# google/deepconsensus

Hardware: NVIDIA H100
Metric: zmw_windows_per_sec (higher is better)
Workload: dtype bf16

## Files before the change

### deepconsensus_b200/csrc/engine.cu

```cuda
#include <cuda_bf16.h>
#include <cuda_runtime.h>
#include <math.h>
#include <stdarg.h>
#include <stdio.h>
#include <string.h>

#include <algorithm>
#include <cmath>
#include <functional>
#include <map>
#include <memory>
#include <string>
#include <vector>

#include "../../include/dcb200.h"
#include "../../include/dcb200_debug.h"
#include "kernels.h"

using namespace dcb;

namespace {

thread_local std::string g_create_error;

// ... 68 lines not shown

enum ProfKind { kProfEmbed, kProfRowGemm, kProfQkv, kProfAttention, kProfFfn, kProfHead, kProfKinds, kProfNone };

struct ProfRegion { cudaEvent_t start, end; ProfKind kind; };

}

struct dcb_engine {
  dcb_config cfg{};
  std::string err;
  int R = 0, L = 0, Lw = 0, E = 0, Epad = 0, echunks = 0;
  PackedLayout pl{};
  int chunk_tiles = 0, chunk_windows = 0;
  int num_sms = 132;
  cudaStream_t stream = nullptr;
  cudaStream_t copy_stream = nullptr;
  cudaStream_t out_stream = nullptr;
  struct Slot {
    DevBuf<float> d_rows;
    DevBuf<uint8_t> d_packed;
    DevBuf<uint8_t> d_bases, d_quals;
    DevBuf<float> d_probs, d_logits;
    DevBuf<int> d_status;
    int* h_status = nullptr;
    cudaEvent_t rows_ready = nullptr, ev0 = nullptr, ev1 = nullptr, done = nullptr;
    bool busy = false, used = false;
    int64_t ticket = -1;
    int launches = 0;
    std::vector<ProfRegion> prof;
    size_t prof_used = 0;
  } slots[2];
  int64_t next_ticket = 0;
  bool weights_loaded = false;
  bool debug = false;
  bool profile = false;
  float prof_ms[kProfKinds] = {};
  int prof_n[kProfKinds] = {};
  long long prof_ffn_tokens = 0;
  float last_ms = 0.f;
  int last_launches = 0;
  int last_chunk_tokens = 0;
  std::vector<EmbedTable> tables;
  std::vector<StrictEmbedRow> embed;
  int table_elems = 0;
  Weights w;
  DevBuf<__nv_bfloat16> d_embqkv;
  DevBuf<float> d_x;
  DevBuf<__nv_bfloat16> d_xb;
  DevBuf<__nv_bfloat16> d_att;
  DevBuf<__nv_bfloat16> d_hid;
  DevBuf<int> d_flow;
  uint32_t flow_stamp = 0;
  bool tile_flow = false;
  DevBuf<double> d_p10;
  DevBuf<float> d_dbg;
  DevBuf<__nv_bfloat16> d_dbg_op;
  struct Strict {
    DevBuf<float> emb, x, y, q, k, v, att, hid;
    int chunk_windows = 0;
  } strict;
  struct {
    DevBuf<uint8_t> bases, quals, seq, qual, names, fastq;
    DevBuf<int32_t> start, len, pos, name_off, outcome;
    DevBuf<int64_t> rec_off, win_off;
    DevBuf<double> avg_q;
  } st;
  struct { DevBuf<int16_t> bq; DevBuf<uint8_t> mask; DevBuf<double> avg; } sk;
  struct {
    DevBuf<uint8_t> ids, bases, quals; DevBuf<int16_t> bq; DevBuf<int32_t> dst; DevBuf<int64_t> src_off, dst_off; DevBuf<int> status;
  } fs;
  struct { DevBuf<float> probs, loss; DevBuf<uint8_t> labels, ccs, exact; DevBuf<int32_t> pred, ccs_counts; DevBuf<int> bad; } ev;
  struct { DevBuf<float> teacher, student, loss, grad; } ds;
  struct { DevBuf<float> probs, loss, grad, matches, dp; DevBuf<uint8_t> labels; } lg;
  struct { DevBuf<float> bias, logits, probs; DevBuf<uint8_t> bases, quals; } he;
  struct {
    DevBuf<PrepZmw> zmw;
    DevBuf<int32_t> meta, noni, gap, zmw_windows, window_pos, window_width, num_passes, list, wl;
    DevBuf<int64_t> ccs_off;
    DevBuf<float> sn;
    DevBuf<uint32_t> cigar;
    DevBuf<uint8_t> bases, pw, ip, ccs_bases, ccs_bq, spaced, overflow, ccs_ids, packed;
    DevBuf<int4> op_scan, zmw_out;
    DevBuf<int4> win_list, window;
    DevBuf<int16_t> out_bq, ccs_bq_full;
    DevBuf<uint8_t> ccs_ids_full;
    DevBuf<int32_t> label_meta;
    DevBuf<uint32_t> label_cigar;
    DevBuf<uint8_t> label_bases, labels, label_status;
    DevBuf<int4> label_scan;
    DevBuf<int32_t> eval_dst;
    DevBuf<uint8_t> keep;
    DevBuf<int> eval_count;
    std::vector<int32_t> width;
    DevBuf<int> status;
    PrepBatch batch{};
    int n_windows = -1;
  } fp;
  cudaEvent_t ev_eval0 = nullptr, ev_eval1 = nullptr;

  ~dcb_engine() {
    for (cudaStream_t s : {copy_stream, stream, out_stream})
      if (s) cudaStreamSynchronize(s);
    std::vector<cudaEvent_t> events = {ev_eval0, ev_eval1};
    for (Slot& sl : slots) {
      events.insert(events.end(), {sl.rows_ready, sl.ev0, sl.ev1, sl.done});
      for (const ProfRegion& r : sl.prof) events.insert(events.end(), {r.start, r.end});
// ... 480 lines not shown
  const uint32_t nstamps = 3 + 3 * (uint32_t)c.num_hidden_layers;
  if (flow && e->flow_stamp > UINT32_MAX - nstamps) {
    cudaMemsetAsync(e->d_flow, 0, e->chunk_tiles * sizeof(int), st);
    e->flow_stamp = 0;
  }
  auto next_flow = [&](bool advance = true) {
    TileFlow f{};
    if (flow) {
      f.flags = e->d_flow;
      f.status = d_status;
      f.wait = (int)e->flow_stamp;
      f.done = (int)(e->flow_stamp + 1);
      if (advance) ++e->flow_stamp;
    }
    return f;
  };
  int stage = 0;
  auto snap = [&]() {
    if (e->debug) {
      const size_t ximg = x_image_elems(), cw = (size_t)e->chunk_tiles * kTileM;
      cudaMemcpyAsync(e->d_dbg + (size_t)stage * e->chunk_tiles * ximg, e->d_x, T * ximg * sizeof(float), cudaMemcpyDeviceToDevice, st);
      size_t cols = 0;
      for (const DbgImage& im : dbg_images(e)) {
        if (im.stage == stage)
          cudaMemcpyAsync(e->d_dbg_op + cols * cw, im.src->p, (size_t)T * kTileM * im.width * sizeof(__nv_bfloat16),
                          cudaMemcpyDeviceToDevice, st);
        cols += im.width;
      }
    }
    ++stage;
  };
  rec.run(kProfEmbed, 1, [&] {
    launch_embed(rows_chunk, packed_chunk, e->pl, e->R, L, Lw, M, T, e->echunks, W.cols, W.rowmeta, W.tables,
                 e->table_elems, e->d_embqkv, d_status, next_flow(), st);
  });
  rec.run(kProfRowGemm, 1, [&] {
    launch_gemm_row(e->d_embqkv, W.wc, e->Epad / 16, 2 * (e->Epad / 16), T, row_epi(e, false, nullptr, 0, 0, true),
                    next_flow(), st);
  });
  snap();
  for (int n_ = 0; n_ < c.num_hidden_layers; ++n_) {
    const LayerDev& ld = W.layers[n_];
    if (Lw == kTileM) {
      rec.run(kProfAttention, 2, [&] {
        __nv_bfloat16* qkv = e->debug ? e->d_embqkv.p : nullptr;
        for (int half = 0; half < 2; ++half)
          launch_qkv_attention(half, e->d_xb, ld.wqkv, L, c.attn_win_size, T, qkv, e->d_att, next_flow(half == 1), st);
      });
    } else {
      rec.run(kProfQkv, 1, [&] { launch_gemm_qkv(e->d_xb, ld.wqkv, T, e->d_embqkv, st); });
      rec.run(kProfAttention, 1, [&] { launch_attention(e->d_embqkv, e->d_att, L, Lw, c.attn_win_size, bw, st); });
    }
    rec.run(kProfRowGemm, 1, [&] {
      launch_gemm_row(e->d_att, ld.wo, kDP / 16, 2 * (kDP / 16), T, row_epi(e, true, nullptr, n_, 1, false), next_flow(),
                      st);
    });
    snap();
    rec.run(kProfFfn, 2, [&] {
      const RowEpi epi = row_epi(e, true, ld.b2, n_ + 1, 0, false);
      __nv_bfloat16* hid = e->debug ? e->d_hid.p : nullptr;
      for (int half = 0; half < 2; ++half)
        launch_ffn(half, e->d_xb, ld.w1, ld.b1, ld.w2, c.filter_size, T, hid, epi, next_flow(half == 1), st);
    });
    if (e->profile) e->prof_ffn_tokens += (long long)bw * L;
    snap();
  }
  hp.x = e->d_x; hp.M = M; hp.L = L; hp.Lw = Lw;
  rec.run(kProfHead, 1, [&] { launch_head(hp, T, next_flow(), st); });
  e->last_chunk_tokens = M;
}

}

extern "C" {

const char* dcb_version(void) { return "dcb200 0.1.0 (sm_90a)"; }

const char* dcb_last_error(const dcb_engine* e) { return e ? e->err.c_str() : g_create_error.c_str(); }

int dcb_create(const dcb_config* cfg, dcb_engine** out) {
  if (!cfg || !out) return fail(nullptr, DCB_ERR_INVALID, "null argument");
  if (cfg->struct_size != (int32_t)sizeof(dcb_config))
    return fail(nullptr, DCB_ERR_INVALID, "dcb_config size mismatch: got %d, built with %zu",
                cfg->struct_size, sizeof(dcb_config));
  if (cfg->hidden_size != kD || cfg->num_heads != kHeads)
    return fail(nullptr, DCB_ERR_INVALID, "unsupported model: hidden_size=%d num_heads=%d (engine is built for %d/%d)",
                cfg->hidden_size, cfg->num_heads, kD, kHeads);
  if (!cfg->condense_transformer_input)
    return fail(nullptr, DCB_ERR_INVALID, "condense_transformer_input must be true");
  if (cfg->filter_size <= 0 || cfg->filter_size % kFFChunk || cfg->filter_size > 2048)
    return fail(nullptr, DCB_ERR_INVALID, "filter_size must be a multiple of %d and <= 2048", kFFChunk);
  if (cfg->max_passes <= 0 || cfg->max_length <= 0 || cfg->max_length > 256 || cfg->num_hidden_layers <= 0 ||
      cfg->max_batch <= 0)
    return fail(nullptr, DCB_ERR_INVALID, "bad max_passes/max_length(<=256)/num_hidden_layers/max_batch");
  if (cfg->precision != DCB_PRECISION_BF16 && cfg->precision != DCB_PRECISION_FP32 && cfg->precision != DCB_PRECISION_TF32X3)
    return fail(nullptr, DCB_ERR_INVALID, "precision must be DCB_PRECISION_BF16, DCB_PRECISION_FP32 or DCB_PRECISION_TF32X3");
  int ndev = 0;
  if (cudaGetDeviceCount(&ndev) != cudaSuccess || ndev == 0)
    return fail(nullptr, DCB_ERR_CUDA, "no CUDA device available (the dcb200 engine has no CPU fallback)");
  if (cfg->device < 0 || cfg->device >= ndev) return fail(nullptr, DCB_ERR_INVALID, "bad device ordinal %d", cfg->device);
  cudaDeviceProp prop;
  if (cudaGetDeviceProperties(&prop, cfg->device) != cudaSuccess || prop.major != 9)
    return fail(nullptr, DCB_ERR_CUDA, "device %d is not an sm_90 GPU (compute capability %d.%d)", cfg->device,
                prop.major, prop.minor);

  std::unique_ptr<dcb_engine> eng(new dcb_engine());
  dcb_engine* e = eng.get();
  e->cfg = *cfg;
  e->num_sms = prop.multiProcessorCount;
  e->L = cfg->max_length;
  e->Lw = e->L;
  bool align = true, tile_flow = true;
#ifdef DCB_DEV_SWITCHES
  if (const char* env = getenv("DCB_ALIGN")) align = atoi(env) != 0;
  if (const char* env = getenv("DCB_TILE_FLOW")) tile_flow = atoi(env) != 0;
#endif
  if (align && e->L <= kTileM) e->Lw = kTileM;
  e->tile_flow = tile_flow && e->Lw == kTileM;
  e->R = 4 * cfg->max_passes + (cfg->use_ccs_bq ? 6 : 5);
  e->pl = make_packed_layout(cfg->max_passes, cfg->max_length, cfg->use_ccs_bq ? 1 : 0);
  {
    auto table = [&](const char* layer, int vocab, int width) {
      const int off = (e->table_elems + 7) / 8 * 8;
      e->tables.push_back(EmbedTable{layer, vocab, width, off});
      e->table_elems = off + vocab * width;
      return e->tables.back();
    };
    auto rows = [&](const EmbedTable& tb, int n, float clip, int shift) {
      for (int r = 0; r < n; ++r) {
        e->embed.push_back(StrictEmbedRow{clip, shift, tb.vocab, tb.width, e->E, tb.off});
        e->E += tb.width;
      }
    };
    const int P = cfg->max_passes;
    const EmbedTable bases = table("bases_embedding_layer", kVocab, cfg->per_base_hidden_size);
    rows(bases, P, 0.f, 0);
    rows(table("pw_embedding_layer", cfg->pw_max + 1, cfg->pw_hidden_size), P, (float)cfg->pw_max, 0);
    rows(table("ip_embedding_layer", cfg->ip_max + 1, cfg->ip_hidden_size), P, (float)cfg->ip_max, 0);
    rows(table("strand_embedding_layer", cfg->strand_max + 1, cfg->strand_hidden_size), P, 0.f, 0);
    rows(bases, 1, 0.f, 0);
    if (cfg->use_ccs_bq)
      rows(table("ccs_base_quality_scores_embedding_layer", cfg->ccs_bq_max, cfg->ccs_bq_hidden_size), 1, 0.f, 1);
    rows(table("sn_embedding_layer", cfg->sn_max + 1, cfg->sn_hidden_size), 4, (float)cfg->sn_max, 0);
  }
  e->Epad = (e->E + 15) / 16 * 16;
  e->echunks = e->Epad / 8;
  const int ct = cfg->chunk_tiles > 0 ? cfg->chunk_tiles : 8 * e->num_sms;
  const int max_tiles = (int)(((int64_t)cfg->max_batch * e->Lw + kTileM - 1) / kTileM);
  e->chunk_windows = std::max(1, std::min(cfg->max_batch, ct * kTileM / e->Lw));
  e->chunk_tiles = std::min(max_tiles, (e->chunk_windows * e->Lw + kTileM - 1) / kTileM);

  const int rc = [&]() -> int {
    CU(e, cudaSetDevice(cfg->device));
    CU(e, cudaStreamCreateWithFlags(&e->stream, cudaStreamNonBlocking));
    CU(e, cudaStreamCreateWithFlags(&e->copy_stream, cudaStreamNonBlocking));
    CU(e, cudaStreamCreateWithFlags(&e->out_stream, cudaStreamNonBlocking));
    for (auto& sl : e->slots) {
      CU(e, cudaEventCreateWithFlags(&sl.rows_ready, cudaEventDisableTiming));
      CU(e, cudaEventCreate(&sl.ev0));
      CU(e, cudaEventCreate(&sl.ev1));
      CU(e, cudaEventCreateWithFlags(&sl.done, cudaEventDisableTiming));
      CU(e, cudaMallocHost(reinterpret_cast<void**>(&sl.h_status), sizeof(int)));
    }
    CU(e, cudaEventCreate(&e->ev_eval0));
    CU(e, cudaEventCreate(&e->ev_eval1));
    CU(e, kernels_init());
    CU(e, tf32x3_init());
    std::vector<double> p10(256);
// ... 1131 lines not shown
```

### deepconsensus_b200/csrc/kernels.cu

```cuda
#include "kernels.h"

#include <cuda_bf16.h>
#include <math.h>
#include <stdio.h>
#include <stdlib.h>

#include "head_finish.cuh"
#include "sm90.cuh"

namespace dcb {

__device__ __forceinline__ void pdl_launch_dependents() { asm volatile("griddepcontrol.launch_dependents;" ::: "memory"); }
__device__ __forceinline__ void pdl_wait() { asm volatile("griddepcontrol.wait;" ::: "memory"); }

__device__ __forceinline__ int ld_acquire_gpu(const int* p) {
  int v;
  asm volatile("ld.acquire.gpu.global.b32 %0, [%1];" : "=r"(v) : "l"(p) : "memory");
  return v;
}

__device__ __forceinline__ void tile_wait(const TileFlow& f, int tile) {
  if (!f.flags) return;
  if (ld_acquire_gpu(f.flags + tile) == f.wait) return;
  uint64_t t0, t;
// ... 80 lines not shown
    uint4* dst = reinterpret_cast<uint4*>(emb + ((size_t)tile * echunks + kc) * kTileM * 8) + r;
    *dst = val;
  }
  __syncthreads();
  if (threadIdx.x == 0) tile_done(flow, tile);
}

enum { EPI_QKV = 0, EPI_ROW = 1 };

template <int BN, int NCH, bool kAres>
struct GemmCfg {
  static constexpr int kNI = NCH * BN;
  static constexpr int kSK = 2;
  static constexpr int kABytesPerK = 2 * kTileM * 16;
  static constexpr int kBBytesPerK = 2 * kNI * 16;
  static constexpr int kStageBytes = kSK * ((kAres ? 0 : kABytesPerK) + kBBytesPerK);
  static constexpr int kStages = 8;
  static constexpr int kShortStages = 4;
  static constexpr int kLongK = 32;
  __host__ __device__ static constexpr int stages(int kstages) {
    return kAres || kstages >= kLongK ? kStages : kShortStages;
  }
  static constexpr int kMH = kAres ? 2 : 1;
  static constexpr int kATileBytes = (kDP / 16) * kABytesPerK;
  static constexpr int kAresBytes = kAres ? 2 * kATileBytes : 0;
  static constexpr int kThreads = 384;
  static constexpr int kVecBytes = kAres ? 0 : 3 * kDP * 4;
  __host__ __device__ static constexpr int smem_bytes(int nst) { return kAresBytes + nst * kStageBytes + 256 + kVecBytes; }
  static constexpr int kSmemBytes = smem_bytes(kStages);
  static_assert(kSmemBytes <= 232448, "over the sm_90 opt-in shared memory per block");
  static_assert((2 * kStages + 4) * 8 <= 256, "the mbarriers (full, empty, a_full, a_empty, turn[2]) fill 256 bytes");
};

template <int BN>
__device__ __forceinline__ void wgmma_bn(float (&d)[BN / 2], uint64_t a, uint64_t b, int acc);
template <>
__device__ __forceinline__ void wgmma_bn<144>(float (&d)[72], uint64_t a, uint64_t b, int acc) { wgmma_m64n144k16(d, a, b, acc); }
template <>
__device__ __forceinline__ void wgmma_bn<128>(float (&d)[64], uint64_t a, uint64_t b, int acc) { wgmma_m64n128k16(d, a, b, acc); }

__device__ __forceinline__ float quad_sum(float v) {
  v += __shfl_xor_sync(0xffffffffu, v, 1);
  v += __shfl_xor_sync(0xffffffffu, v, 2);
  return v;
}

__device__ __forceinline__ void row_vectors_to_smem(float* s_vec, const RowEpi& epi) {
  for (int i = threadIdx.x; i < kDP; i += blockDim.x) {
    if (epi.bias) s_vec[i] = epi.bias[i];
    if (epi.ln_g) { s_vec[kDP + i] = epi.ln_g[i]; s_vec[2 * kDP + i] = epi.ln_b[i]; }
  }
}

template <int BN, int NCH, bool kPe = true>
__device__ __forceinline__ void row_epilogue(float (&acc)[NCH][BN / 2], int tile, int row0, int q, const float* s_vec,
                                             const RowEpi& epi) {
  float* xt = epi.x + (size_t)tile * x_image_elems();
  const int xoff = ((q >> 1) * kTileM + row0) * 4 + 2 * (q & 1);
  const bool ln = epi.ln_g != nullptr;
#pragma unroll
  for (int h = 0; h < 2; ++h) {
    const int row = row0 + 8 * h;
    const int l = (tile * kTileM + row) % epi.L;
    float* xr = xt + xoff + 32 * h;
    const float* per = epi.pe_img ? epi.pe_img + xoff + 32 * h : epi.pe + (size_t)l * kDP + 2 * q;
    const int pe_stride = epi.pe_img ? kTileM : 1;
    float s1 = 0.f;
#pragma unroll
    for (int j = 0; j < NCH; ++j) {
      float2 ld[BN / 8];
      if (epi.has_xold) {
#pragma unroll
        for (int jj = 0; jj < BN / 8; ++jj)
          ld[jj] = *reinterpret_cast<const float2*>(xr + (j * BN + jj * 8) * kTileM);
#pragma unroll
        for (int jj = 0; jj < BN / 8; ++jj) {
          acc[j][jj * 4 + 2 * h] += ld[jj].x;
          acc[j][jj * 4 + 2 * h + 1] += ld[jj].y;
        }
      }
      if (kPe && epi.pe) {
#pragma unroll
        for (int jj = 0; jj < BN / 8; ++jj)
          ld[jj] = __ldg(reinterpret_cast<const float2*>(per + (size_t)(j * BN + jj * 8) * pe_stride));
      }
#pragma unroll
      for (int jj = 0; jj < BN / 8; ++jj) {
        const int col = j * BN + jj * 8 + 2 * q;
        float2 v = make_float2(acc[j][jj * 4 + 2 * h], acc[j][jj * 4 + 2 * h + 1]);
        if (epi.bias) {
          const float2 b = *reinterpret_cast<const float2*>(s_vec + col);
          v.x += b.x; v.y += b.y;
        }
        if (kPe && epi.pe) { v.x += ld[jj].x; v.y += ld[jj].y; }
        v.x = col < kD ? v.x : 0.f;
        v.y = col + 1 < kD ? v.y : 0.f;
        *reinterpret_cast<float2*>(xr + (j * BN + jj * 8) * kTileM) = v;
        acc[j][jj * 4 + 2 * h] = v.x;
        acc[j][jj * 4 + 2 * h + 1] = v.y;
        s1 += v.x + v.y;
      }
    }
    if (!epi.xb) continue;
    float mean = 0.f, rstd = 1.f;
    if (ln) {
      mean = quad_sum(s1) * (1.f / kD);
      float s2 = 0.f;
#pragma unroll
      for (int j = 0; j < NCH; ++j)
#pragma unroll
        for (int jj = 0; jj < BN / 8; ++jj) {
          const int col = j * BN + jj * 8 + 2 * q;
          const float d0 = col < kD ? acc[j][jj * 4 + 2 * h] - mean : 0.f;
          const float d1 = col + 1 < kD ? acc[j][jj * 4 + 2 * h + 1] - mean : 0.f;
          s2 += d0 * d0 + d1 * d1;
        }
      rstd = rsqrtf(quad_sum(s2) * (1.f / kD) + 1e-6f);
    }
    __nv_bfloat16* xb = epi.xb + (size_t)tile * act_image_elems(kDP) + row * 8 + 2 * q;
#pragma unroll
    for (int j = 0; j < NCH; ++j)
#pragma unroll
      for (int jj = 0; jj < BN / 8; ++jj) {
        const int col = j * BN + jj * 8 + 2 * q;
        float v0 = acc[j][jj * 4 + 2 * h], v1 = acc[j][jj * 4 + 2 * h + 1];
        if (ln) {
          v0 = col < kD ? (v0 - mean) * rstd * s_vec[kDP + col] + s_vec[2 * kDP + col] : 0.f;
          v1 = col + 1 < kD ? (v1 - mean) * rstd * s_vec[kDP + col + 1] + s_vec[2 * kDP + col + 1] : 0.f;
        }
        *reinterpret_cast<uint32_t*>(xb + (j * BN + jj * 8) * kTileM) = pack_bf16x2(v0, v1);
      }
  }
#pragma unroll
  for (int j = 0; j < NCH; ++j)
#pragma unroll
    for (int i = 0; i < BN / 2; ++i) acc[j][i] = 0.f;
}

template <int BN, int NCH, int EPI, bool kAres>
__global__ void __launch_bounds__(384, 1)
gemm_kernel(const __nv_bfloat16* __restrict__ a_img, const __nv_bfloat16* __restrict__ b_img, int a_ksteps, int ksteps,
            int ntiles,
            int ngroups, __nv_bfloat16* __restrict__ out_img, int out_chunks, RowEpi epi, TileFlow flow) {
  using Cfg = GemmCfg<BN, NCH, kAres>;
  static_assert(EPI != EPI_ROW || (Cfg::kNI == kDP && !kAres), "row epilogue needs the full 288-wide row");
  extern __shared__ __align__(1024) uint8_t smem[];
  uint8_t* a_res = smem;
  const int kstages = ksteps / Cfg::kSK;
  const int nst = Cfg::stages(kstages);
  uint8_t* stage_base = smem + Cfg::kAresBytes;
  uint64_t* full = reinterpret_cast<uint64_t*>(stage_base + nst * Cfg::kStageBytes);
  uint64_t* empty = full + nst;
  uint64_t* a_full = empty + nst;
  uint64_t* a_empty = a_full + 1;
  uint64_t* turn = a_empty + 1;
  float* s_vec = reinterpret_cast<float*>(stage_base + nst * Cfg::kStageBytes + 256);

  const int warp = threadIdx.x >> 5;
  const int lane = threadIdx.x & 31;
  if constexpr (EPI == EPI_ROW) row_vectors_to_smem(s_vec, epi);
  if (threadIdx.x == 0) {
    for (int i = 0; i < nst; ++i) {
      mbar_init(&full[i], 1);
      mbar_init(&empty[i], 256);
    }
    mbar_init(a_full, 1);
    mbar_init(a_empty, 256);
    mbar_init(&turn[0], 128);
    mbar_init(&turn[1], 128);
    mbar_fence_init();
  }
  __syncthreads();
  pdl_launch_dependents();

  const int nitems = kAres ? (ntiles + 1) / 2 : ntiles * ngroups;
  const int gper = kAres ? ngroups : 1;
  const size_t a_tile_bytes = (size_t)a_ksteps * Cfg::kABytesPerK;
  const size_t b_group_bytes = (size_t)ksteps * Cfg::kBBytesPerK;

  if (warp >= 8) {
    setmaxnreg_dec<40>();
    if (warp == 8 && lane == 0) {
      uint32_t slot = 0, phase = 0, it = 0;
      for (int item = blockIdx.x; item < nitems; item += gridDim.x, ++it) {
        const int tile = kAres ? 2 * item : item / ngroups;
        const uint8_t* a_src = reinterpret_cast<const uint8_t*>(a_img) + tile * a_tile_bytes;
        tile_wait(flow, tile);
        fence_proxy_async();
        if constexpr (kAres) {
// ... 76 lines not shown
          for (int mh = 0; mh < Cfg::kMH; ++mh) {
            const uint64_t adesc = make_kc16_desc(sa + (kAres ? 64 * mh : 64 * wg) * 16, kTileM * 16, 128);
#pragma unroll
            for (int j = 0; j < NCH; ++j) {
              const uint64_t bdesc = make_kc16_desc(sb + kk * Cfg::kBBytesPerK + j * BN * 16, Cfg::kNI * 16, 128);
              wgmma_bn<BN>(accm[mh][j], adesc, bdesc, (s | kk) != 0);
            }
          }
        }
        wgmma_commit();
#pragma unroll
        for (int mh = 0; mh < Cfg::kMH; ++mh)
#pragma unroll
          for (int j = 0; j < NCH; ++j) wgmma_fence_regs(accm[mh][j]);
        wgmma_wait<1>();
        if (s > 0) mbar_arrive(&empty[prev]);
        prev = slot;
        if (++slot == nst) { slot = 0; phase ^= 1; }
      }
      wgmma_wait<0>();
#pragma unroll
      for (int mh = 0; mh < Cfg::kMH; ++mh)
#pragma unroll
        for (int j = 0; j < NCH; ++j) wgmma_fence_regs(accm[mh][j]);
      mbar_arrive(&empty[prev]);
      if (kAres && gi + 1 == gper) mbar_arrive(a_empty);

      if constexpr (kAres) wait_turn();
      if constexpr (EPI == EPI_QKV) {
        __nv_bfloat16* obase = out_img + (size_t)tile * kTileM * out_chunks * 8;
#pragma unroll
        for (int mh = 0; mh < Cfg::kMH; ++mh)
#pragma unroll
          for (int h = 0; h < 2; ++h) {
            const int row = row0 + 64 * mh + 8 * h;
#pragma unroll
            for (int j = 0; j < NCH; ++j)
#pragma unroll
              for (int jj = 0; jj < BN / 8; ++jj) {
                const int col = grp * Cfg::kNI + j * BN + jj * 8 + 2 * q;
                *reinterpret_cast<uint32_t*>(obase + ((size_t)(col >> 3) * kTileM + row) * 8 + (col & 7)) =
                    pack_bf16x2(accm[mh][j][jj * 4 + 2 * h], accm[mh][j][jj * 4 + 2 * h + 1]);
              }
          }
        if constexpr (kAres) pass_turn();
      } else {
        row_epilogue<BN, NCH>(accm[0], tile, row0, q, s_vec, epi);
      }
    }
    if (flow.flags) {
      consumer_bar_sync();
      if (threadIdx.x == 0) tile_done(flow, item);
    }
  }
  pdl_wait();
}

struct FfnCfg {
  static constexpr int kUpK = kDP / 16;
  static constexpr int kDownK = kFFChunk / 16;
  static constexpr int kABytesPerK = 2 * kTileM * 16;
  static constexpr int kW1Bytes = 2 * kFFChunk * 16;
  static constexpr int kW2Bytes = 2 * kDP * 16;
  static constexpr int kStageBytes = kW2Bytes;
  static constexpr int kB1Off = 2 * kW1Bytes;
  static constexpr int kB1Bytes = kFFChunk * 4;
  static constexpr int kStages = 16;
  static constexpr int kATileBytes = kUpK * kABytesPerK;
  static constexpr int kBarBytes = 512;
  static constexpr int kVecBytes = 3 * kDP * 4;
  static constexpr int kSmemBytes = kATileBytes + kStages * kStageBytes + kBarBytes + kVecBytes;
  static constexpr int kThreads = 384;
  static_assert(kSmemBytes <= 232448, "over the sm_90 opt-in shared memory per block");
  static_assert((2 * kStages + 2) * 8 <= kBarBytes, "the mbarriers (full, empty, a_full, a_empty) fit");
  static_assert(kB1Off + kB1Bytes <= kStageBytes && kUpK % 2 == 0, "a stage holds two W1 k-steps and b1");
};

template <bool kHid>
__global__ void __launch_bounds__(384, 1)
ffn_gemm_kernel(const __nv_bfloat16* __restrict__ xb_img, const __nv_bfloat16* __restrict__ w1_img,
                const float* __restrict__ b1, const __nv_bfloat16* __restrict__ w2_img, int ff, int tile_begin,
                int tile_end, __nv_bfloat16* __restrict__ hid, RowEpi epi, TileFlow flow) {
  using Cfg = FfnCfg;
  extern __shared__ __align__(1024) uint8_t smem[];
  uint8_t* a_res = smem;
  uint8_t* stage_base = smem + Cfg::kATileBytes;
  uint64_t* full = reinterpret_cast<uint64_t*>(stage_base + Cfg::kStages * Cfg::kStageBytes);
  uint64_t* empty = full + Cfg::kStages;
  uint64_t* a_full = empty + Cfg::kStages;
  uint64_t* a_empty = a_full + 1;
  float* s_vec = reinterpret_cast<float*>(reinterpret_cast<uint8_t*>(full) + Cfg::kBarBytes);
  const int nch = ff / kFFChunk;

  const int warp = threadIdx.x >> 5;
  const int lane = threadIdx.x & 31;
  row_vectors_to_smem(s_vec, epi);
  if (threadIdx.x == 0) {
    for (int i = 0; i < Cfg::kStages; ++i) {
      mbar_init(&full[i], 1);
      mbar_init(&empty[i], 256);
    }
    mbar_init(a_full, 1);
    mbar_init(a_empty, 256);
    mbar_fence_init();
  }
  __syncthreads();
// ... 548 lines not shown
        const int col = (c0 + u) * 4 + i;
        s1 += ys[i];
        s2 = fmaf(ys[i], ys[i], s2);
        const float4 w0 = *reinterpret_cast<const float4*>(&sGW[col * 8]);
        const float w4 = sGW[col * 8 + 4];
        t[0] = fmaf(ys[i], w0.x, t[0]); t[1] = fmaf(ys[i], w0.y, t[1]); t[2] = fmaf(ys[i], w0.z, t[2]);
        t[3] = fmaf(ys[i], w0.w, t[3]); t[4] = fmaf(ys[i], w4, t[4]);
      }
    }
  }
  const float m1 = s1 * (1.f / kD);
  const float rstd = rsqrtf(fmaxf(s2 * (1.f / kD) - m1 * m1, 0.f) + 1e-6f);
  float lg[kVocab];
#pragma unroll
  for (int j = 0; j < kVocab; ++j) lg[j] = rstd * (t[j] - m1 * sA[j]) + sBj[j];
  head_finish(p, lg, oidx);
}

__global__ void __launch_bounds__(128)
head_kernel(HeadParams p, TileFlow flow) {
  __shared__ __align__(16) float sGW[kD * 8];
  __shared__ float sA[kVocab], sBj[kVocab];
  for (int i = threadIdx.x; i < kD * 2; i += blockDim.x)
    reinterpret_cast<float4*>(sGW)[i] = __ldg(reinterpret_cast<const float4*>(p.gw8) + i);
  if (threadIdx.x < kVocab) { sA[threadIdx.x] = p.ab[threadIdx.x]; sBj[threadIdx.x] = p.ab[8 + threadIdx.x]; }
  if (threadIdx.x == 0) tile_wait(flow, blockIdx.x);
  __syncthreads();
  head_row(p, sGW, sA, sBj, blockIdx.x, threadIdx.x);
  pdl_wait();
}

static int g_num_sms = 0;
static int num_sms() {
  if (!g_num_sms) {
    int dev = 0;
    cudaGetDevice(&dev);
    cudaDeviceGetAttribute(&g_num_sms, cudaDevAttrMultiProcessorCount, dev);
    if (g_num_sms <= 0) g_num_sms = 132;
  }
  return g_num_sms;
}


template <int BN, int NCH, int EPI, bool kAres>
static cudaError_t gemm_init() {
  return cudaFuncSetAttribute(gemm_kernel<BN, NCH, EPI, kAres>, cudaFuncAttributeMaxDynamicSharedMemorySize,
                              GemmCfg<BN, NCH, kAres>::kSmemBytes);
}

cudaError_t kernels_init() {
  cudaError_t e;
  if ((e = gemm_init<kNC, 2, EPI_ROW, false>()) != cudaSuccess) return e;
  if ((e = gemm_init<kNC, 1, EPI_QKV, true>()) != cudaSuccess) return e;
  for (auto fn : {ffn_gemm_kernel<false>, ffn_gemm_kernel<true>})
    if ((e = cudaFuncSetAttribute(fn, cudaFuncAttributeMaxDynamicSharedMemorySize, FfnCfg::kSmemBytes)) != cudaSuccess)
      return e;
  for (auto fn : {qkv_attention_kernel<false>, qkv_attention_kernel<true>})
    if ((e = cudaFuncSetAttribute(fn, cudaFuncAttributeMaxDynamicSharedMemorySize, QkvAttCfg::kSmemBytes)) !=
        cudaSuccess)
      return e;
  e = cudaFuncSetAttribute(embed_rows_kernel, cudaFuncAttributeMaxDynamicSharedMemorySize, 160 * 1024);
  if (e != cudaSuccess) return e;
  e = cudaFuncSetAttribute(band_attention_kernel, cudaFuncAttributeMaxDynamicSharedMemorySize,
                           2 * 256 * kAttStride * 2);
  return e;
}

template <typename... P, typename... A>
static void launch(const TileFlow& flow, void (*kernel)(P...), int grid, int threads, size_t smem, cudaStream_t st,
                   A... args) {
  cudaLaunchAttribute attr{};
  attr.id = cudaLaunchAttributeProgrammaticStreamSerialization;
  attr.val.programmaticStreamSerializationAllowed = 1;
  cudaLaunchConfig_t cfg{};
  cfg.gridDim = dim3(grid);
  cfg.blockDim = dim3(threads);
  cfg.dynamicSmemBytes = smem;
  cfg.stream = st;
  cfg.attrs = flow.flags ? &attr : nullptr;
  cfg.numAttrs = flow.flags ? 1 : 0;
  cudaLaunchKernelEx(&cfg, kernel, args...);
}

size_t embed_smem_bytes(int R, int echunks, int table_elems) {
  return (size_t)((table_elems * 2 + 15) & ~15) + ((echunks * 8 * sizeof(EmbedCol) + 15) & ~(size_t)15) +
         (size_t)R * kTileM * 2;
}

void launch_embed(const float* rows, const uint8_t* packed, const PackedLayout& pl, int R, int L, int Lw, int M, int ntiles, int echunks,
                  const EmbedCol* cols, const EmbedRow* rowmeta, const __nv_bfloat16* tables,
                  int table_elems, __nv_bfloat16* emb, int* status, const TileFlow& flow, cudaStream_t st) {
  embed_rows_kernel<<<ntiles, 256, embed_smem_bytes(R, echunks, table_elems), st>>>(
      rows, packed, pl, R, L, Lw, M, echunks, cols, rowmeta, tables, table_elems, emb, status, flow);
}

void launch_gemm_row(const __nv_bfloat16* a_img, const __nv_bfloat16* b_img, int a_ksteps, int b_ksteps, int ntiles,
                     const RowEpi& epi, const TileFlow& flow, cudaStream_t st) {
  using Cfg = GemmCfg<kNC, 2, false>;
  const int grid = ntiles < num_sms() ? ntiles : num_sms();
  const int smem = Cfg::smem_bytes(Cfg::stages(b_ksteps / Cfg::kSK));
  launch(flow, gemm_kernel<kNC, 2, EPI_ROW, false>, grid, Cfg::kThreads, smem, st, a_img, b_img, a_ksteps, b_ksteps,
         ntiles, 1, (__nv_bfloat16*)nullptr, 0, epi, flow);
}

void launch_gemm_qkv(const __nv_bfloat16* a_img, const __nv_bfloat16* b_img, int ntiles,
                     __nv_bfloat16* qkv_img, cudaStream_t st) {
  using Cfg = GemmCfg<kNC, 1, true>;
  const int npairs = (ntiles + 1) / 2;
  const int grid = npairs < num_sms() ? npairs : num_sms();
  RowEpi none{};
  gemm_kernel<kNC, 1, EPI_QKV, true><<<grid, Cfg::kThreads, Cfg::kSmemBytes, st>>>(
      a_img, b_img, kDP / 16, 2 * (kDP / 16), ntiles, kQKVN / kQKVGroup, qkv_img, kQKVN / 8, none, TileFlow{});
}

void launch_ffn(int half, const __nv_bfloat16* xb_img, const __nv_bfloat16* w1_img, const float* b1,
                const __nv_bfloat16* w2_img, int ff, int ntiles, __nv_bfloat16* hid_img, const RowEpi& epi,
                const TileFlow& flow, cudaStream_t st) {
  const int split = (ntiles + 1) / 2;
  const int t0 = half ? split : 0, t1 = half ? ntiles : split;
  const int n = t1 - t0;
  const int grid = n < 1 ? 1 : n < num_sms() ? n : num_sms();
  launch(flow, hid_img ? ffn_gemm_kernel<true> : ffn_gemm_kernel<false>, grid, FfnCfg::kThreads, FfnCfg::kSmemBytes,
         st, xb_img, w1_img, b1, w2_img, ff, t0, t1, hid_img, epi, flow);
}

__global__ void __launch_bounds__(256)
unpack_rows_kernel(const uint8_t* __restrict__ packed, PackedLayout pl, int nwindows, float* __restrict__ rows) {
  const int b = blockIdx.x;
  const uint8_t* w = packed + (size_t)b * pl.stride;
  float* out = rows + (size_t)b * pl.R * pl.L;
  for (int i = threadIdx.x; i < pl.R * pl.L; i += blockDim.x) {
    const int r = i / pl.L, l = i - r * pl.L;
    out[i] = packed_value(pl, w, r, l);
  }
}

void launch_unpack_rows(const uint8_t* packed, const PackedLayout& pl, int nwindows, float* rows, cudaStream_t st) {
  if (nwindows > 0) unpack_rows_kernel<<<nwindows, 256, 0, st>>>(packed, pl, nwindows, rows);
}


void launch_attention(const __nv_bfloat16* qkv, __nv_bfloat16* att, int L, int Lw, int win, int nwindows,
                      cudaStream_t st) {
  const int Lp = (L + 15) & ~15;
  const size_t smem = (size_t)2 * Lp * kAttStride * 2;
  band_attention_kernel<<<nwindows * 2, 128, smem, st>>>(qkv, att, L, Lw, win, nwindows);
}

void launch_qkv_attention(int half, const __nv_bfloat16* xb_img, const __nv_bfloat16* wqkv, int L, int win,
                          int ntiles, __nv_bfloat16* qkv_img, __nv_bfloat16* att, const TileFlow& flow,
                          cudaStream_t st) {
  const int split = (ntiles + 1) / 2;
  const int t0 = half ? split : 0, t1 = half ? ntiles : split;
  const int n = t1 - t0;
  const int grid = n < 1 ? 1 : n < num_sms() ? n : num_sms();
// ... 71 lines not shown
```

### deepconsensus_b200/csrc/kernels.h

```cpp
#pragma once
#include <cuda_runtime.h>

#include <vector>

#include "common.h"

namespace dcb {

cudaError_t kernels_init();

size_t embed_smem_bytes(int R, int echunks, int table_elems);
void launch_embed(const float* rows, const uint8_t* packed, const PackedLayout& pl, int R, int L, int Lw, int M, int ntiles, int echunks,
                  const EmbedCol* cols, const EmbedRow* rowmeta, const __nv_bfloat16* tables,
                  int table_elems, __nv_bfloat16* emb, int* status, const TileFlow& flow, cudaStream_t st);
void launch_gemm_row(const __nv_bfloat16* a_img, const __nv_bfloat16* b_img, int a_ksteps, int b_ksteps, int ntiles,
                     const RowEpi& epi, const TileFlow& flow, cudaStream_t st);
void launch_gemm_qkv(const __nv_bfloat16* a_img, const __nv_bfloat16* b_img, int ntiles,
                     __nv_bfloat16* qkv_img, cudaStream_t st);
void launch_ffn(int half, const __nv_bfloat16* xb_img, const __nv_bfloat16* w1_img, const float* b1,
                const __nv_bfloat16* w2_img, int ff, int ntiles, __nv_bfloat16* hid_img, const RowEpi& epi,
                const TileFlow& flow, cudaStream_t st);
void launch_unpack_rows(const uint8_t* packed, const PackedLayout& pl, int nwindows, float* rows, cudaStream_t st);
void launch_attention(const __nv_bfloat16* qkv, __nv_bfloat16* att, int L, int Lw, int win, int nwindows,
                      cudaStream_t st);
void launch_qkv_attention(int half, const __nv_bfloat16* xb_img, const __nv_bfloat16* wqkv, int L, int win,
                          int ntiles, __nv_bfloat16* qkv_img, __nv_bfloat16* att, const TileFlow& flow,
                          cudaStream_t st);
void launch_head(const HeadParams& p, int ntiles, const TileFlow& flow, cudaStream_t st);
__host__ __device__ inline int64_t window_offset(const int64_t* win_off, int w, int L) {
  return win_off ? win_off[w] : (int64_t)w * L;
}
void launch_stitch(const uint8_t* bases, const uint8_t* quals, int L, const int64_t* win_off, const int32_t* zmw_start,
                   int n_zmw, uint8_t* seq_out, uint8_t* qual_out, int32_t* len_out, cudaStream_t st);


void launch_read_outcome(const uint8_t* qual, const int32_t* len, const int64_t* win_off, const int32_t* zmw_start,
                         const int32_t* window_pos, int L, int n_zmw, const double* p10, double min_quality, int min_length,
                         int32_t* outcome, double* avg_q, cudaStream_t st);
void launch_fastq(const uint8_t* seq, const uint8_t* qual, const int32_t* len, const int64_t* win_off, const int32_t* zmw_start,
                  int L, int n_zmw, const int32_t* outcome, const uint8_t* names, const int32_t* name_off, int64_t* rec_off,
                  uint8_t* fastq, int64_t cap, cudaStream_t st);
void launch_skip_mask(const int16_t* ccs_bq, int n_windows, int L, const double* p10, double thr, uint8_t* mask,
                      double* avg_out, cudaStream_t st);
void launch_fill_skipped(const uint8_t* ccs_ids, const int16_t* ccs_bq, const int64_t* src_off, const int32_t* dst,
                         const int64_t* dst_off, int k, int L, int64_t total, int calib_enabled, double thr, double cw,
                         double cb, int max_q, uint8_t* bases, uint8_t* quals, int* status, cudaStream_t st);
void launch_head_epilogue(const float* logits, int n, const HeadParams& p, cudaStream_t st);

constexpr int kReadMeta = 10;
struct PrepZmw {
  int32_t read0, n_reads;
  int32_t keep;
  int32_t ccs_off, ccs_len, bq_any;
  int32_t mb;
  int32_t wb;
  int32_t win_off, win_cap;
  int32_t wl_off, wl_n;
  int64_t gap_off;
  int64_t plane_off;
};
struct PrepBatch {
  int n_zmw, ins_trim;
  PackedLayout pl;
  const PrepZmw* zmw;
  const int32_t* read_meta;
  const float* read_sn;
  const uint32_t* cigar;
  const uint8_t *bases, *pw, *ip, *ccs_bases, *ccs_bq;
  const int32_t* wl;
// ... 65 lines not shown
```

### deepconsensus_b200/csrc/sm90.cuh

```cuda
#pragma once
#include <cuda_bf16.h>
#include <cuda_runtime.h>
#include <stdint.h>

namespace dcb {

__device__ __forceinline__ uint32_t smem_u32(const void* p) {
  return static_cast<uint32_t>(__cvta_generic_to_shared(p));
}

__device__ __forceinline__ void mbar_init(uint64_t* bar, uint32_t count) {
  asm volatile("mbarrier.init.shared::cta.b64 [%0], %1;" ::"r"(smem_u32(bar)), "r"(count));
}
__device__ __forceinline__ void mbar_fence_init() {
  asm volatile("fence.mbarrier_init.release.cluster;" ::: "memory");
}
__device__ __forceinline__ void mbar_arrive(uint64_t* bar) {
  asm volatile("{\n\t.reg .b64 st;\n\tmbarrier.arrive.shared::cta.b64 st, [%0];\n\t}" ::"r"(smem_u32(bar)) : "memory");
}
__device__ __forceinline__ void mbar_arrive_expect_tx(uint64_t* bar, uint32_t bytes) {
  asm volatile("{\n\t.reg .b64 st;\n\tmbarrier.arrive.expect_tx.shared::cta.b64 st, [%0], %1;\n\t}" ::"r"(smem_u32(bar)),
               "r"(bytes)
               : "memory");
}
__device__ __forceinline__ void mbar_wait(uint64_t* bar, uint32_t parity) {
  asm volatile(
      "{\n\t.reg .pred p;\n"
      "DCB_MBAR_WAIT:\n\t"
      "mbarrier.try_wait.parity.shared::cta.b64 p, [%0], %1;\n\t"
      "@!p bra DCB_MBAR_WAIT;\n\t}" ::"r"(smem_u32(bar)),
      "r"(parity)
      : "memory");
}

__device__ __forceinline__ void bulk_g2s(void* smem_dst, const void* gmem_src, uint32_t bytes, uint64_t* bar) {
  asm volatile(
      "cp.async.bulk.shared::cluster.global.mbarrier::complete_tx::bytes [%0], [%1], %2, [%3];" ::"r"(
          smem_u32(smem_dst)),
      "l"(gmem_src), "r"(bytes), "r"(smem_u32(bar))
      : "memory");
}

__device__ __forceinline__ uint64_t make_kc16_desc(uint32_t smem_addr, uint32_t lbo_bytes, uint32_t sbo_bytes) {
  uint64_t d = 0;
  d |= static_cast<uint64_t>((smem_addr >> 4) & 0x3FFF);
  d |= static_cast<uint64_t>((lbo_bytes >> 4) & 0x3FFF) << 16;
  d |= static_cast<uint64_t>((sbo_bytes >> 4) & 0x3FFF) << 32;
  return d;
}

__device__ __forceinline__ void wgmma_fence() { asm volatile("wgmma.fence.sync.aligned;" ::: "memory"); }
__device__ __forceinline__ void wgmma_commit() { asm volatile("wgmma.commit_group.sync.aligned;" ::: "memory"); }
template <int N>
__device__ __forceinline__ void wgmma_wait() {
  asm volatile("wgmma.wait_group.sync.aligned %0;" ::"n"(N) : "memory");
}
template <int N>
__device__ __forceinline__ void wgmma_fence_regs(float (&d)[N]) {
#pragma unroll
  for (int i = 0; i < N; ++i) asm volatile("" : "+f"(d[i])::"memory");
}
template <int N>
__device__ __forceinline__ void wgmma_fence_regs(uint32_t (&a)[N]) {
#pragma unroll
  for (int i = 0; i < N; ++i) asm volatile("" : "+r"(a[i])::"memory");
}

__device__ __forceinline__ void wgmma_m64n144k16(float (&d)[72], uint64_t a_desc, uint64_t b_desc, int accumulate) {
  asm volatile(
      "{\n\t.reg .pred p;\n\t"
      "setp.ne.b32 p, %74, 0;\n\t"
      "wgmma.mma_async.sync.aligned.m64n144k16.f32.bf16.bf16 "
      "{%0, %1, %2, %3, %4, %5, %6, %7, %8, %9, %10, %11, %12, %13, %14, %15, %16, %17, %18, %19, %20, %21, %22, %23, %24, %25, %26, %27, %28, %29, %30, %31, %32, %33, %34, %35, %36, %37, %38, %39, %40, %41, %42, %43, %44, %45, %46, %47, %48, %49, %50, %51, %52, %53, %54, %55, %56, %57, %58, %59, %60, %61, %62, %63, %64, %65, %66, %67, %68, %69, %70, %71}, %72, %73, p, 1, 1, 0, 0;\n\t}"
      : "+f"(d[0]), "+f"(d[1]), "+f"(d[2]), "+f"(d[3]), "+f"(d[4]), "+f"(d[5]), "+f"(d[6]), "+f"(d[7]),
        "+f"(d[8]), "+f"(d[9]), "+f"(d[10]), "+f"(d[11]), "+f"(d[12]), "+f"(d[13]), "+f"(d[14]), "+f"(d[15]),
        "+f"(d[16]), "+f"(d[17]), "+f"(d[18]), "+f"(d[19]), "+f"(d[20]), "+f"(d[21]), "+f"(d[22]), "+f"(d[23]),
        "+f"(d[24]), "+f"(d[25]), "+f"(d[26]), "+f"(d[27]), "+f"(d[28]), "+f"(d[29]), "+f"(d[30]), "+f"(d[31]),
        "+f"(d[32]), "+f"(d[33]), "+f"(d[34]), "+f"(d[35]), "+f"(d[36]), "+f"(d[37]), "+f"(d[38]), "+f"(d[39]),
        "+f"(d[40]), "+f"(d[41]), "+f"(d[42]), "+f"(d[43]), "+f"(d[44]), "+f"(d[45]), "+f"(d[46]), "+f"(d[47]),
        "+f"(d[48]), "+f"(d[49]), "+f"(d[50]), "+f"(d[51]), "+f"(d[52]), "+f"(d[53]), "+f"(d[54]), "+f"(d[55]),
        "+f"(d[56]), "+f"(d[57]), "+f"(d[58]), "+f"(d[59]), "+f"(d[60]), "+f"(d[61]), "+f"(d[62]), "+f"(d[63]),
        "+f"(d[64]), "+f"(d[65]), "+f"(d[66]), "+f"(d[67]), "+f"(d[68]), "+f"(d[69]), "+f"(d[70]), "+f"(d[71])
      : "l"(a_desc), "l"(b_desc), "r"(accumulate));
}

__device__ __forceinline__ void wgmma_m64n144k16_rs(float (&d)[72], const uint32_t (&a)[4], uint64_t b_desc,
                                                    int accumulate) {
  asm volatile(
      "{\n\t.reg .pred p;\n\t"
      "setp.ne.b32 p, %77, 0;\n\t"
      "wgmma.mma_async.sync.aligned.m64n144k16.f32.bf16.bf16 "
      "{%0, %1, %2, %3, %4, %5, %6, %7, %8, %9, %10, %11, %12, %13, %14, %15, %16, %17, %18, %19, %20, %21, %22, %23, %24, %25, %26, %27, %28, %29, %30, %31, %32, %33, %34, %35, %36, %37, %38, %39, %40, %41, %42, %43, %44, %45, %46, %47, %48, %49, %50, %51, %52, %53, %54, %55, %56, %57, %58, %59, %60, %61, %62, %63, %64, %65, %66, %67, %68, %69, %70, %71}, {%72, %73, %74, %75}, %76, p, 1, 1, 0;\n\t}"
      : "+f"(d[0]), "+f"(d[1]), "+f"(d[2]), "+f"(d[3]), "+f"(d[4]), "+f"(d[5]), "+f"(d[6]), "+f"(d[7]),
        "+f"(d[8]), "+f"(d[9]), "+f"(d[10]), "+f"(d[11]), "+f"(d[12]), "+f"(d[13]), "+f"(d[14]), "+f"(d[15]),
// ... 61 lines not shown
```

Before: 182,500.

## Add warp-specialized out-projection kernel with TMA-staged residual epilogue

```diff
diff --git a/deepconsensus_b200/csrc/engine.cu b/deepconsensus_b200/csrc/engine.cu
--- a/deepconsensus_b200/csrc/engine.cu
+++ b/deepconsensus_b200/csrc/engine.cu
@@ -144,6 +144,7 @@
   DevBuf<int> d_flow;
   uint32_t flow_stamp = 0;
   bool tile_flow = false;
+  bool outproj = true;
   DevBuf<double> d_p10;
   DevBuf<float> d_dbg;
   DevBuf<__nv_bfloat16> d_dbg_op;
@@ -730,8 +731,9 @@
       rec.run(kProfAttention, 1, [&] { launch_attention(e->d_embqkv, e->d_att, L, Lw, c.attn_win_size, bw, st); });
     }
     rec.run(kProfRowGemm, 1, [&] {
-      launch_gemm_row(e->d_att, ld.wo, kDP / 16, 2 * (kDP / 16), T, row_epi(e, true, nullptr, n_, 1, false), next_flow(),
-                      st);
+      const RowEpi epi = row_epi(e, true, nullptr, n_, 1, false);
+      if (e->outproj) launch_outproj(e->d_att, ld.wo, T, epi, next_flow(), st);
+      else launch_gemm_row(e->d_att, ld.wo, kDP / 16, 2 * (kDP / 16), T, epi, next_flow(), st);
     });
     snap();
     rec.run(kProfFfn, 2, [&] {
@@ -792,6 +794,7 @@
 #ifdef DCB_DEV_SWITCHES
   if (const char* env = getenv("DCB_ALIGN")) align = atoi(env) != 0;
   if (const char* env = getenv("DCB_TILE_FLOW")) tile_flow = atoi(env) != 0;
+  if (const char* env = getenv("DCB_OUTPROJ")) e->outproj = atoi(env) != 0;
 #endif
   if (align && e->L <= kTileM) e->Lw = kTileM;
   e->tile_flow = tile_flow && e->Lw == kTileM;
diff --git a/deepconsensus_b200/csrc/kernels.cu b/deepconsensus_b200/csrc/kernels.cu
--- a/deepconsensus_b200/csrc/kernels.cu
+++ b/deepconsensus_b200/csrc/kernels.cu
@@ -156,17 +156,16 @@
   }
 }
 
-template <int BN, int NCH, bool kPe = true>
-__device__ __forceinline__ void row_epilogue(float (&acc)[NCH][BN / 2], int tile, int row0, int q, const float* s_vec,
-                                             const RowEpi& epi) {
-  float* xt = epi.x + (size_t)tile * x_image_elems();
+template <int BN, int NCH, bool kPe>
+__device__ __forceinline__ void row_epilogue_at(float (&acc)[NCH][BN / 2], int tile, int row0, int q, const float* s_vec,
+                                                const RowEpi& epi, float* xr0, int xstride) {
   const int xoff = ((q >> 1) * kTileM + row0) * 4 + 2 * (q & 1);
   const bool ln = epi.ln_g != nullptr;
 #pragma unroll
   for (int h = 0; h < 2; ++h) {
     const int row = row0 + 8 * h;
     const int l = (tile * kTileM + row) % epi.L;
-    float* xr = xt + xoff + 32 * h;
+    float* xr = xr0 + 32 * h;
     const float* per = epi.pe_img ? epi.pe_img + xoff + 32 * h : epi.pe + (size_t)l * kDP + 2 * q;
     const int pe_stride = epi.pe_img ? kTileM : 1;
     float s1 = 0.f;
@@ -176,7 +175,7 @@
       if (epi.has_xold) {
 #pragma unroll
         for (int jj = 0; jj < BN / 8; ++jj)
-          ld[jj] = *reinterpret_cast<const float2*>(xr + (j * BN + jj * 8) * kTileM);
+          ld[jj] = *reinterpret_cast<const float2*>(xr + (j * BN + jj * 8) * xstride);
 #pragma unroll
         for (int jj = 0; jj < BN / 8; ++jj) {
           acc[j][jj * 4 + 2 * h] += ld[jj].x;
@@ -199,7 +198,7 @@
         if (kPe && epi.pe) { v.x += ld[jj].x; v.y += ld[jj].y; }
         v.x = col < kD ? v.x : 0.f;
         v.y = col + 1 < kD ? v.y : 0.f;
-        *reinterpret_cast<float2*>(xr + (j * BN + jj * 8) * kTileM) = v;
+        *reinterpret_cast<float2*>(xr + (j * BN + jj * 8) * xstride) = v;
         acc[j][jj * 4 + 2 * h] = v.x;
         acc[j][jj * 4 + 2 * h + 1] = v.y;
         s1 += v.x + v.y;
@@ -239,6 +238,13 @@
   for (int j = 0; j < NCH; ++j)
 #pragma unroll
     for (int i = 0; i < BN / 2; ++i) acc[j][i] = 0.f;
+}
+
+template <int BN, int NCH, bool kPe = true>
+__device__ __forceinline__ void row_epilogue(float (&acc)[NCH][BN / 2], int tile, int row0, int q, const float* s_vec,
+                                             const RowEpi& epi) {
+  float* xr0 = epi.x + (size_t)tile * x_image_elems() + ((q >> 1) * kTileM + row0) * 4 + 2 * (q & 1);
+  row_epilogue_at<BN, NCH, kPe>(acc, tile, row0, q, s_vec, epi, xr0, kTileM);
 }
 
 template <int BN, int NCH, int EPI, bool kAres>
@@ -421,6 +427,155 @@
       consumer_bar_sync();
       if (threadIdx.x == 0) tile_done(flow, item);
     }
+  }
+  pdl_wait();
+}
+
+struct OutProjCfg {
+  static constexpr int kK = kDP / 16;
+  static constexpr int kABytesPerK = 2 * kTileM * 16;
+  static constexpr int kATileBytes = kK * kABytesPerK;
+  static constexpr int kBBytesPerK = 2 * kDP * 16;
+  static constexpr int kStageBytes = kABytesPerK + kBBytesPerK;
+  static constexpr int kStages = 5;
+  static constexpr int kRunBytes = 64 * 4 * 4;
+  static constexpr int kOddOff = kRunBytes + 64;
+  static constexpr int kPairBytes = kRunBytes + kOddOff;
+  static constexpr int kXBytes = kXChunks / 2 * kPairBytes;
+  static constexpr int kXStride = kPairBytes / 32;
+  static constexpr int kBarBytes = 128;
+  static constexpr int kVecBytes = 3 * kDP * 4;
+  static constexpr int kSmemBytes = 2 * kXBytes + kStages * kStageBytes + kBarBytes + kVecBytes;
+  static constexpr int kThreads = 384;
+  static_assert(kSmemBytes <= 232448, "over the sm_90 opt-in shared memory per block");
+  static_assert((2 * kStages + 4) * 8 <= kBarBytes, "the mbarriers (full, empty, x_full[2], x_ready[2]) fit");
+  static_assert(kPairBytes % 32 == 0 && kXBytes % 16 == 0, "column stride in floats; 16-byte aligned copies");
+};
+
+__device__ __forceinline__ int outproj_staged_off(int chunk) {
+  return (chunk >> 1) * OutProjCfg::kPairBytes + (chunk & 1) * OutProjCfg::kOddOff;
+}
+
+__global__ void __launch_bounds__(384, 1)
+outproj_kernel(const __nv_bfloat16* __restrict__ att, const __nv_bfloat16* __restrict__ wo, int ntiles, RowEpi epi,
+               TileFlow flow) {
+  using Cfg = OutProjCfg;
+  extern __shared__ __align__(1024) uint8_t smem[];
+  uint8_t* xs = smem;
+  uint8_t* ring = smem + 2 * Cfg::kXBytes;
+  uint64_t* full = reinterpret_cast<uint64_t*>(ring + Cfg::kStages * Cfg::kStageBytes);
+  uint64_t* empty = full + Cfg::kStages;
+  uint64_t* x_full = empty + Cfg::kStages;
+  uint64_t* x_ready = x_full + 2;
+  float* s_vec = reinterpret_cast<float*>(reinterpret_cast<uint8_t*>(full) + Cfg::kBarBytes);
+
+  const int warp = threadIdx.x >> 5;
+  const int lane = threadIdx.x & 31;
+  row_vectors_to_smem(s_vec, epi);
+  if (threadIdx.x == 0) {
+    for (int i = 0; i < Cfg::kStages; ++i) {
+      mbar_init(&full[i], 1);
+      mbar_init(&empty[i], 256);
+    }
+    for (int h = 0; h < 2; ++h) {
+      mbar_init(&x_full[h], 1);
+      mbar_init(&x_ready[h], 128);
+    }
+    mbar_fence_init();
+  }
+  __syncthreads();
+  pdl_launch_dependents();
+
+  if (warp >= 8) {
+    setmaxnreg_dec<40>();
+    if (warp == 8 && lane == 0) {
+      uint32_t slot = 0, phase = 0;
+      for (int tile = blockIdx.x; tile < ntiles; tile += gridDim.x) {
+        const uint8_t* a_src = reinterpret_cast<const uint8_t*>(att) + (size_t)tile * Cfg::kATileBytes;
+        tile_wait(flow, tile);
+        fence_proxy_async();
+        for (int s = 0; s < 2 * Cfg::kK; ++s) {
+          mbar_wait(&empty[slot], phase ^ 1);
+          uint8_t* st = ring + slot * Cfg::kStageBytes;
+          mbar_arrive_expect_tx(&full[slot], Cfg::kStageBytes);
+          bulk_g2s(st, a_src + (size_t)(s % Cfg::kK) * Cfg::kABytesPerK, Cfg::kABytesPerK, &full[slot]);
+          bulk_g2s(st + Cfg::kABytesPerK, reinterpret_cast<const uint8_t*>(wo) + (size_t)s * Cfg::kBBytesPerK,
+                   Cfg::kBBytesPerK, &full[slot]);
+          if (++slot == Cfg::kStages) { slot = 0; phase ^= 1; }
+        }
+      }
+    } else if (warp == 9 && lane == 0) {
+      float* const x = epi.x;
+      auto load_tile = [&](int tile) {
+        tile_wait(flow, tile);
+        fence_proxy_async();
+        for (int h = 0; h < 2; ++h) {
+          const float* src = x + (size_t)tile * x_image_elems() + 64 * h * 4;
+          mbar_arrive_expect_tx(&x_full[h], kXChunks * Cfg::kRunBytes);
+#pragma unroll 4
+          for (int c = 0; c < kXChunks; ++c)
+            bulk_g2s(xs + h * Cfg::kXBytes + outproj_staged_off(c), src + (size_t)c * kTileM * 4, Cfg::kRunBytes,
+                     &x_full[h]);
+        }
+      };
+      if ((int)blockIdx.x < ntiles) load_tile(blockIdx.x);
+      uint32_t it = 0;
+      for (int tile = blockIdx.x; tile < ntiles; tile += gridDim.x, ++it) {
+        for (int h = 0; h < 2; ++h) {
+          mbar_wait(&x_ready[h], it & 1);
+          float* dst = x + (size_t)tile * x_image_elems() + 64 * h * 4;
+#pragma unroll 4
+          for (int c = 0; c < kXChunks; ++c)
+            bulk_s2g(dst + (size_t)c * kTileM * 4, xs + h * Cfg::kXBytes + outproj_staged_off(c), Cfg::kRunBytes);
+          bulk_commit();
+        }
+        bulk_wait_read<0>();
+        const int next = tile + gridDim.x;
+        if (next < ntiles) load_tile(next);
+        bulk_wait<0>();
+        fence_proxy_async();
+        tile_done(flow, tile);
+      }
+    }
+    return;
+  }
+
+  setmaxnreg_inc<232>();
+  const int wg = warp >> 2;
+  const int g = lane >> 2, q = lane & 3;
+  const int lrow0 = (warp & 3) * 16 + g;
+  const int row0 = wg * 64 + lrow0;
+  float* xs0 = reinterpret_cast<float*>(xs + wg * Cfg::kXBytes + (q >> 1) * Cfg::kOddOff) + lrow0 * 4 + 2 * (q & 1);
+  float acc[2][kNC / 2];
+  uint32_t slot = 0, phase = 0, it = 0;
+  for (int tile = blockIdx.x; tile < ntiles; tile += gridDim.x, ++it) {
+    uint32_t prev = 0;
+    for (int s = 0; s < 2 * Cfg::kK; ++s) {
+      mbar_wait(&full[slot], phase);
+      const uint32_t st = smem_u32(ring + slot * Cfg::kStageBytes);
+      wgmma_fence_regs(acc[0]);
+      wgmma_fence_regs(acc[1]);
+      wgmma_fence();
+      const uint64_t adesc = make_kc16_desc(st + 64 * wg * 16, kTileM * 16, 128);
+#pragma unroll
+      for (int j = 0; j < 2; ++j)
+        wgmma_m64n144k16(acc[j], adesc, make_kc16_desc(st + Cfg::kABytesPerK + j * kNC * 16, kDP * 16, 128), s != 0);
+      wgmma_commit();
+      wgmma_fence_regs(acc[0]);
+      wgmma_fence_regs(acc[1]);
+      wgmma_wait<1>();
+      if (s > 0) mbar_arrive(&empty[prev]);
+      prev = slot;
+      if (++slot == Cfg::kStages) { slot = 0; phase ^= 1; }
+    }
+    wgmma_wait<0>();
+    wgmma_fence_regs(acc[0]);
+    wgmma_fence_regs(acc[1]);
+    mbar_arrive(&empty[prev]);
+    mbar_wait(&x_full[wg], it & 1);
+    row_epilogue_at<kNC, 2, false>(acc, tile, row0, q, s_vec, epi, xs0, Cfg::kXStride);
+    fence_proxy_async_smem();
+    mbar_arrive(&x_ready[wg]);
   }
   pdl_wait();
 }
@@ -1075,6 +1230,9 @@
   cudaError_t e;
   if ((e = gemm_init<kNC, 2, EPI_ROW, false>()) != cudaSuccess) return e;
   if ((e = gemm_init<kNC, 1, EPI_QKV, true>()) != cudaSuccess) return e;
+  if ((e = cudaFuncSetAttribute(outproj_kernel, cudaFuncAttributeMaxDynamicSharedMemorySize, OutProjCfg::kSmemBytes)) !=
+      cudaSuccess)
+    return e;
   for (auto fn : {ffn_gemm_kernel<false>, ffn_gemm_kernel<true>})
     if ((e = cudaFuncSetAttribute(fn, cudaFuncAttributeMaxDynamicSharedMemorySize, FfnCfg::kSmemBytes)) != cudaSuccess)
       return e;
@@ -1124,6 +1282,12 @@
   const int smem = Cfg::smem_bytes(Cfg::stages(b_ksteps / Cfg::kSK));
   launch(flow, gemm_kernel<kNC, 2, EPI_ROW, false>, grid, Cfg::kThreads, smem, st, a_img, b_img, a_ksteps, b_ksteps,
          ntiles, 1, (__nv_bfloat16*)nullptr, 0, epi, flow);
+}
+
+void launch_outproj(const __nv_bfloat16* att, const __nv_bfloat16* wo, int ntiles, const RowEpi& epi,
+                    const TileFlow& flow, cudaStream_t st) {
+  const int grid = ntiles < num_sms() ? ntiles : num_sms();
+  launch(flow, outproj_kernel, grid, OutProjCfg::kThreads, OutProjCfg::kSmemBytes, st, att, wo, ntiles, epi, flow);
 }
 
 void launch_gemm_qkv(const __nv_bfloat16* a_img, const __nv_bfloat16* b_img, int ntiles,
diff --git a/deepconsensus_b200/csrc/kernels.h b/deepconsensus_b200/csrc/kernels.h
--- a/deepconsensus_b200/csrc/kernels.h
+++ b/deepconsensus_b200/csrc/kernels.h
@@ -15,6 +15,8 @@
                   int table_elems, __nv_bfloat16* emb, int* status, const TileFlow& flow, cudaStream_t st);
 void launch_gemm_row(const __nv_bfloat16* a_img, const __nv_bfloat16* b_img, int a_ksteps, int b_ksteps, int ntiles,
                      const RowEpi& epi, const TileFlow& flow, cudaStream_t st);
+void launch_outproj(const __nv_bfloat16* att, const __nv_bfloat16* wo, int ntiles, const RowEpi& epi,
+                    const TileFlow& flow, cudaStream_t st);
 void launch_gemm_qkv(const __nv_bfloat16* a_img, const __nv_bfloat16* b_img, int ntiles,
                      __nv_bfloat16* qkv_img, cudaStream_t st);
 void launch_ffn(int half, const __nv_bfloat16* xb_img, const __nv_bfloat16* w1_img, const float* b1,
diff --git a/deepconsensus_b200/csrc/sm90.cuh b/deepconsensus_b200/csrc/sm90.cuh
--- a/deepconsensus_b200/csrc/sm90.cuh
+++ b/deepconsensus_b200/csrc/sm90.cuh
@@ -40,6 +40,21 @@
       "l"(gmem_src), "r"(bytes), "r"(smem_u32(bar))
       : "memory");
 }
+__device__ __forceinline__ void bulk_s2g(void* gmem_dst, const void* smem_src, uint32_t bytes) {
+  asm volatile("cp.async.bulk.global.shared::cta.bulk_group [%0], [%1], %2;" ::"l"(gmem_dst), "r"(smem_u32(smem_src)),
+               "r"(bytes)
+               : "memory");
+}
+__device__ __forceinline__ void bulk_commit() { asm volatile("cp.async.bulk.commit_group;" ::: "memory"); }
+template <int N>
+__device__ __forceinline__ void bulk_wait_read() {
+  asm volatile("cp.async.bulk.wait_group.read %0;" ::"n"(N) : "memory");
+}
+template <int N>
+__device__ __forceinline__ void bulk_wait() {
+  asm volatile("cp.async.bulk.wait_group %0;" ::"n"(N) : "memory");
+}
+__device__ __forceinline__ void fence_proxy_async_smem() { asm volatile("fence.proxy.async.shared::cta;" ::: "memory"); }
 
 __device__ __forceinline__ uint64_t make_kc16_desc(uint32_t smem_addr, uint32_t lbo_bytes, uint32_t sbo_bytes) {
   uint64_t d = 0;
```

New measurement: 184,500 (median of 6 runs). 1.01x the previous value.
